# wusize/CLIPSelf

Measured on AMD Instinct MI355X. Metric: images/sec (student+teacher distill step), ViT-B/16 32 crops/img, higher is better.
Workload: dtype bf16; 1 GPU; EVA02-CLIP-B-16 CLIPSelf image-patches step, 64 images x 32 crops per GPU, 224^2 (BASELINE configs[1]); global_batch=64, crops_per_image=32, image_size=224, parallelism=dp1, teacher_chunk=2048, teacher_last_block=cls_query_only, teacher_schedule=one_batch_ahead_on_side_stream

## Files before the change

clipself_amd/csrc/gemm_stream.hip:

```cpp
#include <vector>
#include <cstdio>
#include "gemm_common.h"

namespace {

typedef __attribute__((ext_vector_type(2))) unsigned u32x2;
typedef __attribute__((ext_vector_type(4))) unsigned u32x4;

constexpr unsigned OOB = 0xfffffff0u;

__device__ __forceinline__ float lane_bcast(int src_lane_x4, float v) {
    return __int_as_float(__builtin_amdgcn_ds_bpermute(src_lane_x4, __float_as_int(v)));
}
__device__ __forceinline__ unsigned pack2(float a, float b) {
    union { bf16x2 v; unsigned u; } pk;
    pk.v[0] = f2bf(a);
    pk.v[1] = f2bf(b);
    return pk.u;
}
__device__ __forceinline__ void swap32(unsigned& x, unsigned& y) {
    const u32x2 r = __builtin_amdgcn_permlane32_swap(x, y, false, false);
    x = r[0];
    y = r[1];
}
__device__ __forceinline__ float both_halves(float v) {
    const u32x2 r = __builtin_amdgcn_permlane32_swap(__float_as_uint(v), __float_as_uint(v), false, false);
    return __uint_as_float(r[0]) + __uint_as_float(r[1]);
}
__device__ __forceinline__ __amdgpu_buffer_rsrc_t make_rsrc(const void* base) {
    return __builtin_amdgcn_make_buffer_rsrc(const_cast<void*>(base), 0, 0x7fffffff, 0x00020000);
}
template <int CP>
__device__ __forceinline__ void store16(const u32x4& v, __amdgpu_buffer_rsrc_t rs, unsigned off) {
    __builtin_amdgcn_raw_buffer_store_b128(v, rs, off, 0, CP);
}
template <int CP>
__device__ __forceinline__ void store8(const u32x2& v, __amdgpu_buffer_rsrc_t rs, unsigned off) {
    __builtin_amdgcn_raw_buffer_store_b64(v, rs, off, 0, CP);
}
__device__ __forceinline__ float dot2_bf16(unsigned a, unsigned b, float c) {
    return __builtin_amdgcn_fdot2_f32_bf16(__builtin_bit_cast(bf16x2, a), __builtin_bit_cast(bf16x2, b), c, false);
}
__device__ __forceinline__ float silu_mul(float u, float v) {
    return u * __builtin_amdgcn_rcpf(1.f + __builtin_amdgcn_exp2f(-1.4426950408889634f * u)) * v;
}
template <int ACT>
__device__ __forceinline__ float activate_s(float v) {
    if (ACT == 1) return 0.5f * v * (1.f + erff(v * 0.70710678118654752f));
    if (ACT == 2) return v * __builtin_amdgcn_rcpf(1.f + __builtin_amdgcn_exp2f(-1.702f * 1.4426950408889634f * v));
    return v;
}

struct EpiOps {
    float mean[4], rstd[4];
    float cb, cc;
};

template <bool LN, bool AUX, int CP, int FM = 4>
__device__ __forceinline__ void epi_swiglu(const GemmArgs& p, const f32x16 (&acc)[FM][2], int lane, int row0, int tn, int wn, const EpiOps& eo) {
    const int l31 = lane & 31, hf = lane >> 5;
    const int hbase = tn * 128 + wn * 32;
    const bool colok = hbase < p.group;
    float nm[FM], rs[FM];
#pragma unroll
    for (int i = 0; i < FM; ++i) {
        rs[i] = LN ? eo.rstd[i] : 1.f;
        nm[i] = LN ? -eo.rstd[i] * eo.mean[i] : 0.f;
    }
    unsigned pk[FM][4][2];
    float ssum[4] = {0.f, 0.f, 0.f, 0.f}, ssq[4] = {0.f, 0.f, 0.f, 0.f};
    const int sl0 = hf << 4;
#pragma unroll
    for (int q = 0; q < 4; ++q) {
        float hv[FM][4];
#pragma unroll
        for (int r = 0; r < 4; ++r) {
            const int e = q * 4 + r;
            const int sl = sl0 + ((8 * q + r) << 2);
            const float b1 = lane_bcast(sl, eo.cb), b2 = lane_bcast(sl + 128, eo.cb);
            float c1 = 0.f, c2 = 0.f;
            if (LN) { c1 = lane_bcast(sl, eo.cc); c2 = lane_bcast(sl + 128, eo.cc); }
#pragma unroll
            for (int i = 0; i < FM; ++i) {
                float u = acc[i][0][e], v = acc[i][1][e];
                if (LN) {
                    u = fmaf(rs[i], u, fmaf(nm[i], c1, b1));
                    v = fmaf(rs[i], v, fmaf(nm[i], c2, b2));
                } else {
                    u += b1;
                    v += b2;
                }
                hv[i][r] = silu_mul(u, v);
            }
        }
#pragma unroll
        for (int i = 0; i < FM; ++i) {
            pk[i][q][0] = pack2(hv[i][0], hv[i][1]);
            pk[i][q][1] = pack2(hv[i][2], hv[i][3]);
            if (AUX) {
#pragma unroll
                for (int d = 0; d < 2; ++d) {
                    ssum[i] = dot2_bf16(pk[i][q][d], 0x3f803f80u, ssum[i]);
                    ssq[i] = dot2_bf16(pk[i][q][d], pk[i][q][d], ssq[i]);
                }
            }
        }
    }
    const __amdgpu_buffer_rsrc_t rc = make_rsrc((const __bf16*)p.C + (size_t)row0 * p.ldc + hbase);
#pragma unroll
    for (int i = 0; i < FM; ++i) {
        const bool ok = colok && row0 + i * 32 + l31 < p.M && !CS_ABL(p, 8);
        const unsigned rowoff = (unsigned)((i * 32 + l31) * p.ldc + 8 * hf) * 2u;
#pragma unroll
        for (int pr = 0; pr < 2; ++pr) {
            unsigned x0 = pk[i][2 * pr][0], x1 = pk[i][2 * pr][1], y0 = pk[i][2 * pr + 1][0], y1 = pk[i][2 * pr + 1][1];
            swap32(x0, y0);
            swap32(x1, y1);
            store16<CP>(u32x4{x0, x1, y0, y1}, rc, ok ? rowoff + 32u * pr : OOB);
        }
    }
    if (AUX) {
        const size_t slice = (size_t)tn * 4 + wn;
        const __amdgpu_buffer_rsrc_t rst = make_rsrc(p.stats_part + (slice * p.M + row0) * 2);
#pragma unroll
        for (int i = 0; i < FM; ++i) {
            const float s = both_halves(ssum[i]), q2 = both_halves(ssq[i]);
            const bool ok = colok && hf == 0 && row0 + i * 32 + l31 < p.M;
            store8<CP>(u32x2{__float_as_uint(s), __float_as_uint(q2)}, rst, ok ? (unsigned)(i * 32 + l31) * 8u : OOB);
        }
    }
}

template <int ACT, bool LN, int CP, bool F8 = false, int FM = 4>
__device__ __forceinline__ void epi_bf16(const GemmArgs& p, const f32x16 (&acc)[FM][2], int lane, int row0, int colw, const EpiOps& eo) {
    const int l31 = lane & 31, hf = lane >> 5;
    float nm[FM], rs[FM];
#pragma unroll
    for (int i = 0; i < FM; ++i) {
        rs[i] = (LN || F8) ? eo.rstd[i] : 1.f;
        nm[i] = LN ? -eo.rstd[i] * eo.mean[i] : 0.f;
    }
    const __amdgpu_buffer_rsrc_t rc = make_rsrc((const __bf16*)p.C + (size_t)row0 * p.ldc + colw);
    const int sl0 = hf << 4;
    unsigned pk[2][FM][4][2];
#pragma unroll
    for (int j = 0; j < 2; ++j) {
#pragma unroll
        for (int q = 0; q < 4; ++q) {
            float ov[FM][4];
#pragma unroll
            for (int r = 0; r < 4; ++r) {
                const int sl = sl0 + ((j * 32 + 8 * q + r) << 2);
                const float b = lane_bcast(sl, eo.cb);
                const float c = (LN || F8) ? lane_bcast(sl, eo.cc) : 0.f;
#pragma unroll
                for (int i = 0; i < FM; ++i) {
                    const float a = acc[i][j][q * 4 + r];
                    ov[i][r] = activate_s<ACT>(F8 ? fmaf(rs[i] * c, a, b) : LN ? fmaf(rs[i], a, fmaf(nm[i], c, b)) : a + b);
                }
            }
#pragma unroll
            for (int i = 0; i < FM; ++i) {
                pk[j][i][q][0] = pack2(ov[i][0], ov[i][1]);
                pk[j][i][q][1] = pack2(ov[i][2], ov[i][3]);
            }
        }
    }
#pragma unroll
    for (int i = 0; i < FM; ++i) {
        const bool rowok = row0 + i * 32 + l31 < p.M && !CS_ABL(p, 8);
#pragma unroll
        for (int j = 0; j < 2; ++j) {
            const bool ok = rowok && colw + j * 32 < p.N;
            const unsigned rowoff = (unsigned)((i * 32 + l31) * p.ldc + j * 32 + 8 * hf) * 2u;
#pragma unroll
            for (int pr = 0; pr < 2; ++pr) {
                unsigned x0 = pk[j][i][2 * pr][0], x1 = pk[j][i][2 * pr][1], y0 = pk[j][i][2 * pr + 1][0], y1 = pk[j][i][2 * pr + 1][1];
                swap32(x0, y0);
                swap32(x1, y1);
                store16<CP>(u32x4{x0, x1, y0, y1}, rc, ok ? rowoff + 32u * pr : OOB);
            }
        }
    }
}


template <int ACT, bool LN, int CP>
__device__ __forceinline__ void epi_bf16_slab(const GemmArgs& p, const f32x16 (&acc)[4][2], int lane, int row0, int colw, const EpiOps& eo, char* slab) {
    const int l31 = lane & 31, hf = lane >> 5;
    float nm[4], rs[4];
#pragma unroll
    for (int i = 0; i < 4; ++i) {
        rs[i] = LN ? eo.rstd[i] : 1.f;
        nm[i] = LN ? -eo.rstd[i] * eo.mean[i] : 0.f;
    }
    const __amdgpu_buffer_rsrc_t rc = make_rsrc((const __bf16*)p.C + (size_t)row0 * p.ldc + colw);
    const int sl0 = hf << 4;
    const int piece = lane & 7, col = colw + piece * 8;
#pragma unroll
    for (int half = 0; half < 2; ++half) {
#pragma unroll
        for (int j = 0; j < 2; ++j)
#pragma unroll
            for (int q = 0; q < 4; ++q) {
                float bq[4], cq[4];
#pragma unroll
                for (int r = 0; r < 4; ++r) {
                    const int sl = sl0 + ((j * 32 + 8 * q + r) << 2);
                    bq[r] = lane_bcast(sl, eo.cb);
                    cq[r] = LN ? lane_bcast(sl, eo.cc) : 0.f;
                }
#pragma unroll
                for (int ii = 0; ii < 2; ++ii) {
                    const int i = half * 2 + ii, lrow = ii * 32 + l31;
                    float ov[4];
#pragma unroll
                    for (int r = 0; r < 4; ++r) {
                        const float a = acc[i][j][q * 4 + r];
                        ov[r] = activate_s<ACT>(LN ? fmaf(rs[i], a, fmaf(nm[i], cq[r], bq[r])) : a + bq[r]);
                    }
                    const int s8 = (j * 8 + 2 * q + hf) ^ ((lrow & 7) << 1);
                    *(uint2*)(slab + lrow * 128 + s8 * 8) = make_uint2(pack2(ov[0], ov[1]), pack2(ov[2], ov[3]));
                }
            }
#pragma unroll
        for (int k = 0; k < 8; ++k) {
            const int lrow = (lane >> 3) + 8 * k, rrel = half * 64 + lrow;
            const uint4 w = *(const uint4*)(slab + lrow * 128 + ((piece ^ (lrow & 7)) << 4));
            const bool ok = row0 + rrel < p.M && col < p.N && !CS_ABL(p, 8);
            store16<CP>(u32x4{w.x, w.y, w.z, w.w}, rc, ok ? (unsigned)(rrel * p.ldc + piece * 8) * 2u : OOB);
        }
    }
}

template <bool LN, bool AUX, int CP>
__device__ __forceinline__ void epi_swiglu_slab(const GemmArgs& p, const f32x16 (&acc)[4][2], int lane, int row0, int tn, int wn, const EpiOps& eo,
                                                char* slab) {
    const int l31 = lane & 31, hf = lane >> 5;
    const int hbase = tn * 128 + wn * 32;
    const bool colok = hbase < p.group;
    float nm[4], rs[4];
#pragma unroll
    for (int i = 0; i < 4; ++i) {
        rs[i] = LN ? eo.rstd[i] : 1.f;
        nm[i] = LN ? -eo.rstd[i] * eo.mean[i] : 0.f;
    }
    float ssum[4] = {0.f, 0.f, 0.f, 0.f}, ssq[4] = {0.f, 0.f, 0.f, 0.f};
    const int sl0 = hf << 4;
#pragma unroll
    for (int q = 0; q < 4; ++q) {
        float hv[4][4];
#pragma unroll
        for (int r = 0; r < 4; ++r) {
            const int e = q * 4 + r;
            const int sl = sl0 + ((8 * q + r) << 2);
            const float b1 = lane_bcast(sl, eo.cb), b2 = lane_bcast(sl + 128, eo.cb);
            float c1 = 0.f, c2 = 0.f;
            if (LN) { c1 = lane_bcast(sl, eo.cc); c2 = lane_bcast(sl + 128, eo.cc); }
#pragma unroll
            for (int i = 0; i < 4; ++i) {
                float u = acc[i][0][e], v = acc[i][1][e];
                if (LN) {
                    u = fmaf(rs[i], u, fmaf(nm[i], c1, b1));
                    v = fmaf(rs[i], v, fmaf(nm[i], c2, b2));
// ... 86 lines not shown
                    xin[it][w >> 1][2 * (w & 1)] = __uint_as_float(__builtin_amdgcn_perm(h[w], l[w], 0x05040100u) - 0x8000u);
                    xin[it][w >> 1][2 * (w & 1) + 1] = __uint_as_float(__builtin_amdgcn_perm(h[w], l[w], 0x07060302u) - 0x8000u);
                }
            } else {
                const unsigned off = ok ? (unsigned)(rrel * p.ldc + piece * 8) * 4u : OOB;
                xin[it][0] = __builtin_bit_cast(f32x4, __builtin_amdgcn_raw_buffer_load_b128(rx, off, 0, CP));
                xin[it][1] = __builtin_bit_cast(f32x4, __builtin_amdgcn_raw_buffer_load_b128(rx, ok ? off + 16u : OOB, 0, CP));
            }
        }
        const float rs_row = (LN || F8) ? eo.rstd[i] : 1.f, nm_row = LN ? -eo.rstd[i] * eo.mean[i] : 0.f;
#pragma unroll
        for (int j = 0; j < 2; ++j)
#pragma unroll
            for (int q = 0; q < 4; ++q) {
                f32x4 t;
#pragma unroll
                for (int r = 0; r < 4; ++r) t[r] = acc[i][j][q * 4 + r];
                const int s16 = (j * 8 + 2 * q + hf) ^ (l31 & 15);
                *(f32x4*)(slab + l31 * 256 + s16 * 16) = t;
            }
        EPI_TRACE(1 + 3 * i);
        EPI_TRACE_WAIT();
        EPI_TRACE(2 + 3 * i);
        const int sel = lane & 7;
        float st_s = 0.f, st_q = 0.f;
#pragma unroll
        for (int it = 0; it < 4; ++it) {
            const int lrow = rrow + 8 * it, rrel = i * 32 + lrow;
            const bool ok = colok && row0 + rrel < p.M;
            float rs = 1.f, nm = 0.f;
            if (LN || F8) rs = lane_bcast(lrow << 2, rs_row);
            if (LN) nm = lane_bcast(lrow << 2, nm_row);
            f32x4 o[2];
#pragma unroll
            for (int h = 0; h < 2; ++h) {
                const f32x4 sv = *(const f32x4*)(slab + lrow * 256 + (((2 * piece + h) ^ (lrow & 15)) << 4));
                if (LN) {
#pragma unroll
                    for (int t = 0; t < 4; ++t) o[h][t] = xin[it][h][t] + fmaf(rs, sv[t], fmaf(nm, cc4[h][t], cb4[h][t]));
                } else if (F8) {
#pragma unroll
                    for (int t = 0; t < 4; ++t) o[h][t] = xin[it][h][t] + fmaf(rs * cc4[h][t], sv[t], cb4[h][t]);
                } else {
                    o[h] = xin[it][h] + (sv + cb4[h]);
                }
            }
            if constexpr (SPLIT & 2) {
                const unsigned off = ok ? (unsigned)(rrel * p.ldxb + piece * 8) * 2u : OOB;
                unsigned y[8];
#pragma unroll
                for (int t = 0; t < 8; ++t) y[t] = __float_as_uint(o[t >> 2][t & 3]) + 0x8000u;
                store16<CP>(u32x4{__builtin_amdgcn_perm(y[1], y[0], 0x07060302u), __builtin_amdgcn_perm(y[3], y[2], 0x07060302u),
                                  __builtin_amdgcn_perm(y[5], y[4], 0x07060302u), __builtin_amdgcn_perm(y[7], y[6], 0x07060302u)}, rb, off);
                store16<CP>(u32x4{__builtin_amdgcn_perm(y[1], y[0], 0x05040100u), __builtin_amdgcn_perm(y[3], y[2], 0x05040100u),
                                  __builtin_amdgcn_perm(y[5], y[4], 0x05040100u), __builtin_amdgcn_perm(y[7], y[6], 0x05040100u)}, rl, off);
            } else {
                const unsigned off = ok ? (unsigned)(rrel * p.ldc + piece * 8) * 4u : OOB;
                store16<CP>(__builtin_bit_cast(u32x4, o[0]), rc, off);
                store16<CP>(__builtin_bit_cast(u32x4, o[1]), rc, ok ? off + 16u : OOB);
            }
            if (AUX) {
                if constexpr (!(SPLIT & 2))
                    store16<CP>(u32x4{pack2(o[0][0], o[0][1]), pack2(o[0][2], o[0][3]), pack2(o[1][0], o[1][1]), pack2(o[1][2], o[1][3])}, rb,
                                ok ? (unsigned)(rrel * p.ldxb + piece * 8) * 2u : OOB);
                float ps = 0.f, pq = 0.f;
                if (colok) {
#pragma unroll
                    for (int t = 0; t < 8; ++t) { ps += o[t >> 2][t & 3]; pq = fmaf(o[t >> 2][t & 3], o[t >> 2][t & 3], pq); }
                }
                const float a = sum_lanes8(ps), b = sum_lanes8(pq);
                if (sel == it) { st_s = a; st_q = b; }
            }
        }
        if (AUX) {
            const int rrel = i * 32 + rrow + 8 * sel;
            const bool ok = sel < 4 && row0 + rrel < p.M && colw < p.N;
            store8<CP>(u32x2{__float_as_uint(st_s), __float_as_uint(st_q)}, rst, ok ? (unsigned)rrel * 8u : OOB);
        }
        EPI_TRACE(3 + 3 * i);
        __builtin_amdgcn_sched_barrier(0);
    }
}

template <int EPI, bool AUX, bool SLAB, int SPLIT = 0, int FM = 4>
constexpr int epi_stores() {
    if (EPI == EPI_SWIGLU_BF16) return FM * (2 + (AUX ? 1 : 0));
    if (EPI == EPI_RESID_F32) return FM * (8 + (AUX ? ((SPLIT & 2) ? 0 : 4) + 1 : 0));
    return FM * 4;
}

#ifndef CS_DMA_AUX_A
#define CS_DMA_AUX_A 0
#endif
#ifndef CS_DMA_AUX_B
#define CS_DMA_AUX_B 0
#endif
#define CS_VMCNT(N) asm volatile("s_waitcnt vmcnt(%0)" ::"n"(N) : "memory")

inline bool getenv_flag(const char* name) {
    const char* v = getenv(name);
    return v && v[0] && v[0] != '0';
}

template <int EPI, bool LN, bool AUX, bool SLAB, bool F8 = false, int SPLIT = 0, int BMT = 256>
__global__ __launch_bounds__(512) void gemm_stream_kernel(GemmArgs p) {
    static_assert(BMT == 256 || (BMT == 192 && !F8 && SPLIT == 0 && !LN && !AUX), "192-row tiles: the training schedule's plain epilogues");
    static_assert(SPLIT == 0 || (EPI == EPI_RESID_F32 && LN && !F8), "the split stream belongs to the folded-LayerNorm residual epilogue");
    static_assert(SLAB || EPI != EPI_RESID_F32, "the fp32 residual epilogue exists in the slab form only (whole-line traffic)");
    static_assert(!F8 || (!LN && !AUX && (EPI == EPI_BF16 || EPI == EPI_RESID_F32)), "fp8 operands: bf16 and fp32-residual outputs");
    constexpr int ES = F8 ? 1 : 2;
    constexpr int CP = 0;
    constexpr bool SWI = EPI == EPI_SWIGLU_BF16, RES = EPI == EPI_RESID_F32;
    static_assert(SWI || RES || epi_is_bf16(EPI), "register epilogues");
    constexpr int BM = BMT, BN = 256, WN = 4, TM = BM / 2, TN = 64, FM = TM / 32, FN = 2;
    constexpr int A_BYTES = BM * BK * 2, B_BYTES = BN * BK * 2;
    constexpr int NPA = BM / 32;
    constexpr int NM = FM * FN, NR = FM + FN;
    constexpr int S = epi_stores<EPI, AUX, SLAB, SPLIT, FM>() < 55 ? epi_stores<EPI, AUX, SLAB, SPLIT, FM>() : 55;
    extern __shared__ __attribute__((aligned(16))) char smem[];
    const int tid = threadIdx.x, lane = tid & 63;
    const int wave = __builtin_amdgcn_readfirstlane(tid >> 6);
    const int wm = wave / WN, wn = wave - wm * WN;
    const int hf = lane >> 5, l31 = lane & 31;
    char* const b_ring = smem + 3 * A_BYTES;
    const int ntiles = p.tiles_m * p.tiles_n, ktiles = p.K / (F8 ? 128 : BK);
    const int a_base = ((wm * TM + l31) >> 1) << 8, b_base = ((wn * TN + l31) >> 1) << 8;
    const int par8 = (l31 & 1) << 3, sw = l31 >> 1;
    const int G = gridDim.x;
#ifndef CS_NO_DMA_ROLES
    constexpr bool ROLES = !F8;
#else
    constexpr bool ROLES = false;
#endif
    const bool role_a = ROLES && wave >= 4;
#ifndef CS_NO_MID_BARRIER
    constexpr bool MID = ROLES && !SLAB && !F8;
#else
    constexpr bool MID = false;
#endif

    unsigned avoff[ROLES ? 8 : 4], bvoff[ROLES ? 1 : 4];
    const char *a_src = nullptr, *b_src = nullptr;
    int a_tile = blockIdx.x, a_kt = 0, b_tile = blockIdx.x, b_kt = 0;
    auto set_a = [&](int tile) {
        int tm, tn;
        tile_of_id(p, tile, ntiles, tm, tn);
        a_src = (const char*)p.A + (size_t)tm * BM * p.lda * ES;
#pragma unroll
        for (int i = 0; i < (ROLES ? NPA : 4); ++i) {
            int tr, chk;
            lane_source(ROLES ? (wave & 3) * NPA + i : wave * 4 + i, lane, tr, chk);
            avoff[i] = (unsigned)(min(tr, p.M - 1 - tm * BM) * p.lda * ES + chk * 16);
        }
    };
    auto set_b = [&](int tile) {
        int tm, tn;
        tile_of_id(p, tile, ntiles, tm, tn);
        if (SWI) {
            b_src = (const char*)p.B + (size_t)tn * (BN / 2) * p.ldb * ES;
        } else {
            b_src = (const char*)p.B + (size_t)tn * BN * p.ldb * ES;
        }
#pragma unroll
        for (int i = 0; i < (ROLES ? 8 : 4); ++i) {
            int tr, chk;
            lane_source(ROLES ? (wave & 3) * 8 + i : wave * 4 + i, lane, tr, chk);
            int rel;
            if (SWI) {
                const int hrel = (tr >> 6) * 32 + (tr & 31);
                rel = ((tr >> 5) & 1) * p.group + min(hrel, p.group - 1 - tn * (BN / 2));
            } else {
                rel = min(tr, p.N - 1 - tn * BN);
            }
            (ROLES ? avoff : bvoff)[i] = (unsigned)(rel * p.ldb * ES + chk * 16);
        }
    };
    auto adv_a = [&]() {
        if (++a_kt == ktiles) {
            a_kt = 0;
            if (a_tile + G < ntiles) {
                a_tile += G;
                set_a(a_tile);
            }
        }
    };
    auto adv_b = [&]() {
        if (++b_kt == ktiles) {
            b_kt = 0;
            if (b_tile + G < ntiles) {
                b_tile += G;
                set_b(b_tile);
            }
        }
    };
#define ISSUE_A(X, SLOT)                                                                                                      \
    __builtin_amdgcn_global_load_lds((const __attribute__((address_space(1))) void*)(a_src + (size_t)a_kt * (BK * 2) + avoff[X]), \
                                     (__attribute__((address_space(3))) void*)(smem + (SLOT) * A_BYTES + (wave * 4 + (X)) * 1024), 16, 0, CS_DMA_AUX_A)
#define ISSUE_B(X, SLOT)                                                                                                      \
    __builtin_amdgcn_global_load_lds((const __attribute__((address_space(1))) void*)(b_src + (size_t)b_kt * (BK * 2) + bvoff[X]), \
                                     (__attribute__((address_space(3))) void*)(b_ring + (SLOT) * B_BYTES + (wave * 4 + (X)) * 1024), 16, 0, CS_DMA_AUX_B)

#define ISSUE_RA(X, SLOT)                                                                                                     \
    __builtin_amdgcn_global_load_lds((const __attribute__((address_space(1))) void*)(a_src + (size_t)a_kt * (BK * 2) + avoff[X]), \
                                     (__attribute__((address_space(3))) void*)(smem + (SLOT) * A_BYTES + ((wave & 3) * NPA + (X)) * 1024), 16, 0, CS_DMA_AUX_A)
#define ISSUE_RB(X, SLOT)                                                                                                     \
    __builtin_amdgcn_global_load_lds((const __attribute__((address_space(1))) void*)(b_src + (size_t)b_kt * (BK * 2) + avoff[X]), \
                                     (__attribute__((address_space(3))) void*)(b_ring + (SLOT) * B_BYTES + ((wave & 3) * 8 + (X)) * 1024), 16, 0, CS_DMA_AUX_B)

    if constexpr (ROLES) {
        if (role_a) {
            set_a(a_tile);
#pragma unroll
            for (int x = 0; x < NPA; ++x) ISSUE_RA(x, 0);
            adv_a();
#pragma unroll
            for (int x = 0; x < NPA; ++x) ISSUE_RA(x, 1);
            adv_a();
        } else {
            set_b(b_tile);
#pragma unroll
            for (int x = 0; x < 8; ++x) ISSUE_RB(x, 0);
            adv_b();
            if constexpr (MID) {
#pragma unroll
                for (int x = 0; x < 8; ++x) ISSUE_RB(x, 1);
                adv_b();
            }
        }
        if constexpr (MID) {
            if (role_a) CS_VMCNT(NPA);
            else CS_VMCNT(8);
            __builtin_amdgcn_s_barrier();
        }
    } else {
        set_a(a_tile);
        set_b(b_tile);
#pragma unroll
        for (int x = 0; x < 4; ++x) ISSUE_A(x, 0);
        adv_a();
#pragma unroll
        for (int x = 0; x < 4; ++x) ISSUE_B(x, 0);
        adv_b();
#pragma unroll
        for (int x = 0; x < 4; ++x) ISSUE_A(x, 1);
        adv_a();
    }

    int curA = 0, gpar = 0;
    bool after_epi = false;
    for (int tile = blockIdx.x; tile < ntiles; tile += G) {
        int tm, tn;
        tile_of_id(p, tile, ntiles, tm, tn);
        const int row0 = tm * BM + wm * TM, colw = tn * BN + wn * TN;
        f32x16 acc[FM][FN];
        EpiOps eo;
        auto load_epi_ops = [&](int ln) {
            const int l31 = ln & 31, hf = ln >> 5, lane = ln;
#pragma unroll
            for (int i = 0; i < 4; ++i) eo.mean[i] = eo.rstd[i] = 0.f;
            eo.cb = eo.cc = 0.f;
            if (LN || F8) {
#pragma unroll
                for (int i = 0; i < FM; ++i) {
                    const int r = min(row0 + i * 32 + l31, p.M - 1);
                    if (LN) eo.mean[i] = p.ln_mean[r];
                    eo.rstd[i] = p.ln_rstd[r];
                }
            }
            int co;
            if (SWI) co = hf * p.group + min(tn * 128 + wn * 32 + l31, p.group - 1);
            else co = min(colw + lane, p.N - 1);
            if (!RES) {
                if (p.bias) eo.cb = p.bias[co];
                if (LN || F8) eo.cc = p.ln_colsum[co];
            }
        };

        auto ktile = [&](auto zero_tag, auto role_tag) {
            constexpr bool ZERO = decltype(zero_tag)::value;
            constexpr int ROLE = decltype(role_tag)::value;
            constexpr int KEEP = ROLE == 0 ? 4 : ROLE == 1 ? 0 : NPA;
            constexpr int SS = S + KEEP > 63 ? 63 - KEEP : S;
            if (after_epi) CS_VMCNT(KEEP + SS);
            else CS_VMCNT(KEEP);
            after_epi = false;
            asm volatile("s_waitcnt lgkmcnt(0)" ::: "memory");
            if (!CS_ABL(p, 2))
                __builtin_amdgcn_s_barrier();
            const char* la = smem + curA * A_BYTES + a_base;
            const char* lb = b_ring + gpar * B_BYTES + b_base;
            const int slot_a2 = curA == 0 ? 2 : curA - 1, slot_b1 = gpar ^ 1;
            if constexpr (F8) {
                typedef __attribute__((ext_vector_type(8))) int i32x8;
                typedef __attribute__((ext_vector_type(4))) int i32x4;
#pragma unroll
                for (int s2 = 0; s2 < 2; ++s2) {
                    const int c0 = 4 * s2 + 2 * hf;
                    const int off0 = ((par8 | c0) ^ sw) << 4, off1 = ((par8 | (c0 + 1)) ^ sw) << 4;
                    i32x8 a8[FM], b8[FN];
#pragma unroll
                    for (int i = 0; i < FM; ++i) {
                        const i32x4 lo = *(const i32x4*)(la + i * (16 * 256) + off0), hi = *(const i32x4*)(la + i * (16 * 256) + off1);
                        a8[i] = i32x8{lo[0], lo[1], lo[2], lo[3], hi[0], hi[1], hi[2], hi[3]};
                    }
#pragma unroll
                    for (int j = 0; j < FN; ++j) {
                        const i32x4 lo = *(const i32x4*)(lb + j * (16 * 256) + off0), hi = *(const i32x4*)(lb + j * (16 * 256) + off1);
                        b8[j] = i32x8{lo[0], lo[1], lo[2], lo[3], hi[0], hi[1], hi[2], hi[3]};
                    }
                    if constexpr (ROLE == 1) {
                        if (s2 == 0) {
#pragma unroll
                            for (int x = 0; x < 8; ++x) ISSUE_RB(x, slot_b1);
                        }
                    } else if constexpr (ROLE == 2) {
                        if (s2 == 1) {
#pragma unroll
                            for (int x = 0; x < NPA; ++x) ISSUE_RA(x, slot_a2);
                        }
                    } else if (s2 == 0) {
                        ISSUE_B(0, slot_b1); ISSUE_B(1, slot_b1); ISSUE_B(2, slot_b1); ISSUE_B(3, slot_b1);
                    } else {
                        ISSUE_A(0, slot_a2); ISSUE_A(1, slot_a2); ISSUE_A(2, slot_a2); ISSUE_A(3, slot_a2);
                    }
#pragma unroll
                    for (int i = 0; i < FM; ++i)
#pragma unroll
                        for (int j = 0; j < FN; ++j) {
                            if (ZERO && s2 == 0) {
                                const f32x16 z = {0.f, 0.f, 0.f, 0.f, 0.f, 0.f, 0.f, 0.f, 0.f, 0.f, 0.f, 0.f, 0.f, 0.f, 0.f, 0.f};
                                acc[i][j] = __builtin_amdgcn_mfma_scale_f32_32x32x64_f8f6f4(b8[j], a8[i], z, 0, 0, 0, 0x7f7f7f7f, 0, 0x7f7f7f7f);
                            } else {
                                acc[i][j] = __builtin_amdgcn_mfma_scale_f32_32x32x64_f8f6f4(b8[j], a8[i], acc[i][j], 0, 0, 0, 0x7f7f7f7f, 0, 0x7f7f7f7f);
                            }
                        }
                }
            } else {
                bf16x8 a[2][FM], b[2][FN];
                auto frags = [&](int ks, int buf) {
                    const int off = ((par8 | (ks * 2 + hf)) ^ sw) << 4;
#pragma unroll
                    for (int i = 0; i < FM; ++i) a[buf][i] = *(const bf16x8*)(la + i * (16 * 256) + off);
#pragma unroll
                    for (int j = 0; j < FN; ++j) b[buf][j] = *(const bf16x8*)(lb + j * (16 * 256) + off);
                };
                frags(0, 0);
#ifndef CS_NO_SGB
                __builtin_amdgcn_sched_group_barrier(0x100, 6, 0);
#endif
#pragma unroll
                for (int ks = 0; ks < 4; ++ks) {
                    const int cb = ks & 1;
                    if (ks < 3) frags(ks + 1, cb ^ 1);
// ... 61 lines not shown
            const char* lb = b_ring + gpar * B_BYTES + b_base;
            const char* la_n = smem + nextA * A_BYTES + a_base;
            const char* lb_n = b_ring + (gpar ^ 1) * B_BYTES + b_base;
            const int slot_a2 = curA == 0 ? 2 : curA - 1, slot_b2 = gpar;
            auto frags = [&](const char* pa, const char* pb, int ks, int buf) {
                const int off = ((par8 | (ks * 2 + hf)) ^ sw) << 4;
#pragma unroll
                for (int i = 0; i < FM; ++i) fa[buf][i] = *(const bf16x8*)(pa + i * (16 * 256) + off);
#pragma unroll
                for (int j = 0; j < FN; ++j) fb[buf][j] = *(const bf16x8*)(pb + j * (16 * 256) + off);
            };
            auto mfmas = [&](int cb, bool zero) {
#pragma unroll
                for (int i = 0; i < FM; ++i)
#pragma unroll
                    for (int j = 0; j < FN; ++j) {
                        if (zero) {
                            const f32x16 z = {0.f, 0.f, 0.f, 0.f, 0.f, 0.f, 0.f, 0.f, 0.f, 0.f, 0.f, 0.f, 0.f, 0.f, 0.f, 0.f};
                            acc[i][j] = __builtin_amdgcn_mfma_f32_32x32x16_bf16(fb[cb][j], fa[cb][i], z, 0, 0, 0);
                        } else {
                            acc[i][j] = __builtin_amdgcn_mfma_f32_32x32x16_bf16(fb[cb][j], fa[cb][i], acc[i][j], 0, 0, 0);
                        }
                    }
            };
            if (ZERO) {
                frags(la, lb, 0, 0);
                __builtin_amdgcn_sched_group_barrier(0x100, 6, 0);
            }
#pragma unroll
            for (int ks = 0; ks < 3; ++ks) {
                const int cb = ks & 1;
                frags(la, lb, ks + 1, cb ^ 1);
                constexpr int KA = 1;
                if constexpr (ROLE == 2) {
                    if (ks == KA) {
#pragma unroll
                        for (int x = 0; x < NPA / 2; ++x) ISSUE_RA(x, slot_a2);
                    }
                    if (ks == KA + 1) {
#pragma unroll
                        for (int x = NPA / 2; x < NPA; ++x) ISSUE_RA(x, slot_a2);
                    }
                }
                mfmas(cb, ZERO && ks == 0);
#pragma unroll
                for (int m = 0; m < NM; ++m) {
                    __builtin_amdgcn_sched_group_barrier(0x008, 1, 0);
                    if (m < NR) __builtin_amdgcn_sched_group_barrier(0x100, 1, 0);
                    if (ROLE == 2 && (ks == KA || ks == KA + 1) && m == NM - 2) __builtin_amdgcn_sched_group_barrier(0x010, 2, 0);
                    if (ROLE == 2 && (ks == KA || ks == KA + 1) && m == NM - 1) __builtin_amdgcn_sched_group_barrier(0x010, NPA / 2 - 2, 0);
                }
            }
            {
                constexpr int KEEP = ROLE == 1 ? 0 : NPA;
                constexpr int SS = S + KEEP > 63 ? 63 - KEEP : S;
                if (after_epi) CS_VMCNT(KEEP + SS);
                else CS_VMCNT(KEEP);
                after_epi = false;
                asm volatile("s_waitcnt lgkmcnt(0)" ::: "memory");
                __builtin_amdgcn_s_barrier();
            }
            {
                const int off = ((par8 | hf) ^ sw) << 4;
#pragma unroll
                for (int x = 0; x < 8; ++x) {
                    if (x < FM) fa[0][x] = *(const bf16x8*)(la_n + x * (16 * 256) + off);
                    else if (x < NR) fb[0][x - FM] = *(const bf16x8*)(lb_n + (x - FM) * (16 * 256) + off);
                    if constexpr (ROLE == 1) ISSUE_RB(x, slot_b2);
                }
            }
            mfmas(1, false);
#pragma unroll
            for (int m = 0; m < NM; ++m) {
                __builtin_amdgcn_sched_group_barrier(0x008, 1, 0);
                if (m < NR) __builtin_amdgcn_sched_group_barrier(0x100, 1, 0);
                if (ROLE == 1 && m < NM - 1) __builtin_amdgcn_sched_group_barrier(0x010, 1, 0);
                if (ROLE == 1 && m == NM - 1) __builtin_amdgcn_sched_group_barrier(0x010, 1 + 8 - NM, 0);
            }
            if (ROLE == 1) adv_b();
            else adv_a();
            curA = nextA;
            gpar ^= 1;
        };
        if constexpr (MID) {
            if (role_a) {
                ktile_mid(std::true_type{}, std::integral_constant<int, 2>{});
                for (int kt = 1; kt < ktiles; ++kt) ktile_mid(std::false_type{}, std::integral_constant<int, 2>{});
            } else {
                ktile_mid(std::true_type{}, std::integral_constant<int, 1>{});
                for (int kt = 1; kt < ktiles; ++kt) ktile_mid(std::false_type{}, std::integral_constant<int, 1>{});
            }
        } else if constexpr (ROLES) {
            if (role_a) {
                ktile(std::true_type{}, std::integral_constant<int, 2>{});
                for (int kt = 1; kt < ktiles; ++kt) ktile(std::false_type{}, std::integral_constant<int, 2>{});
            } else {
                ktile(std::true_type{}, std::integral_constant<int, 1>{});
                for (int kt = 1; kt < ktiles; ++kt) ktile(std::false_type{}, std::integral_constant<int, 1>{});
            }
        } else {
            ktile(std::true_type{}, std::integral_constant<int, 0>{});
            for (int kt = 1; kt < ktiles; ++kt) ktile(std::false_type{}, std::integral_constant<int, 0>{});
        }
        if (CS_ABL(p, 4)) continue;
        after_epi = true;
        int lane_e = lane;
        asm volatile("" : "+v"(lane_e));
        if constexpr (SLAB) {
            asm volatile("s_waitcnt lgkmcnt(0)" ::: "memory");
            __builtin_amdgcn_s_barrier();
            char* const slab = wave >= 4 ? b_ring + (gpar ^ 1) * B_BYTES + (wave - 4) * 8192
                               : (BM == 192 && wave == 3) ? b_ring + 2 * B_BYTES
                                                          : smem + (curA == 0 ? 2 : curA - 1) * A_BYTES + wave * 8192;
            load_epi_ops(lane_e);
#ifndef CS_NO_KERNARG_RELOAD
            constexpr bool RELOAD = RES && LN && AUX;
#else
            constexpr bool RELOAD = false;
#endif
            if constexpr (RELOAD) {
                const __attribute__((address_space(4))) GemmArgs* pk = (const __attribute__((address_space(4))) GemmArgs*)__builtin_amdgcn_kernarg_segment_ptr();
                asm volatile("" : "+s"(pk));
                GemmArgs pe;
                pe.A = pk->A; pe.C = pk->C; pe.bias = pk->bias; pe.extra = pk->extra; pe.M = pk->M; pe.N = pk->N; pe.ldc = pk->ldc;
                pe.ln_colsum = pk->ln_colsum; pe.stats_part = pk->stats_part; pe.xb_out = pk->xb_out; pe.ldxb = pk->ldxb; pe.lo = pk->lo;
                pe.dbg = pk->dbg;
                epi_resid_slab<LN, AUX, CP, F8, SPLIT, FM>(pe, acc, lane_e, row0, colw, tn, wn, eo, slab);
            } else if constexpr (RES) {
                epi_resid_slab<LN, AUX, CP, F8, SPLIT, FM>(p, acc, lane_e, row0, colw, tn, wn, eo, slab);
            } else {
                static_assert(FM == 4, "the slab forms of the bf16 / SwiGLU epilogues exist for 256-row tiles");
                if constexpr (SWI) epi_swiglu_slab<LN, AUX, CP>(p, acc, lane_e, row0, tn, wn, eo, slab);
                else epi_bf16_slab<epi_act(EPI), LN, CP>(p, acc, lane_e, row0, colw, eo, slab);
            }
        } else {
            load_epi_ops(lane_e);
            if constexpr (SWI) epi_swiglu<LN, AUX, CP, FM>(p, acc, lane_e, row0, tn, wn, eo);
            else epi_bf16<epi_act(EPI), LN, CP, F8, FM>(p, acc, lane_e, row0, colw, eo);
        }
    }
    CS_VMCNT(0);
#undef ISSUE_A
#undef ISSUE_B
#undef ISSUE_RA
#undef ISSUE_RB
}

template <int EPI, bool LN, bool AUX, bool SLAB, int BMT = 256>
int launch_stream_v(const GemmArgs& a, unsigned grid, hipStream_t stream) {
    constexpr size_t lds = 160 * 1024;
    static bool once = ((void)hipFuncSetAttribute((const void*)gemm_stream_kernel<EPI, LN, AUX, SLAB, false, 0, BMT>, hipFuncAttributeMaxDynamicSharedMemorySize, (int)lds), true);
    (void)once;
    hipLaunchKernelGGL((gemm_stream_kernel<EPI, LN, AUX, SLAB, false, 0, BMT>), dim3(grid), dim3(512), lds, stream, a);
    CS_LAUNCH_CHECK();
    return 0;
}

template <int EPI, bool LN, bool AUX>
int launch_stream_t(const GemmArgs& a, unsigned grid, hipStream_t stream) {
    if constexpr (EPI == EPI_RESID_F32) return launch_stream_v<EPI, LN, AUX, true>(a, grid, stream);
    else return (a.dbg & 1) ? launch_stream_v<EPI, LN, AUX, true>(a, grid, stream) : launch_stream_v<EPI, LN, AUX, false>(a, grid, stream);
}

template <bool AUX, int SPLIT>
int launch_stream_split(const GemmArgs& a, unsigned grid, hipStream_t stream) {
    constexpr size_t lds = 160 * 1024;
    static bool once = ((void)hipFuncSetAttribute((const void*)gemm_stream_kernel<EPI_RESID_F32, true, AUX, true, false, SPLIT>,
                                                  hipFuncAttributeMaxDynamicSharedMemorySize, (int)lds), true);
    (void)once;
    hipLaunchKernelGGL((gemm_stream_kernel<EPI_RESID_F32, true, AUX, true, false, SPLIT>), dim3(grid), dim3(512), lds, stream, a);
    CS_LAUNCH_CHECK();
    return 0;
}

template <int EPI>
int launch_stream_bf16(const GemmArgs& a, unsigned grid, hipStream_t stream) {
    return a.ln_mean ? launch_stream_t<EPI, true, false>(a, grid, stream) : launch_stream_t<EPI, false, false>(a, grid, stream);
}

template <int EPI, bool SLAB>
int launch_stream_f8(const GemmArgs& a, unsigned grid, hipStream_t stream) {
    constexpr size_t lds = 160 * 1024;
    static bool once = ((void)hipFuncSetAttribute((const void*)gemm_stream_kernel<EPI, false, false, SLAB, true>, hipFuncAttributeMaxDynamicSharedMemorySize, (int)lds), true);
    (void)once;
    hipLaunchKernelGGL((gemm_stream_kernel<EPI, false, false, SLAB, true>), dim3(grid), dim3(512), lds, stream, a);
    CS_LAUNCH_CHECK();
    return 0;
}

}

int cs_gemm_stream_launch_f8(GemmArgs a, int epi, int reserve, hipStream_t stream) {
    a.tiles_m = (a.M + 255) / 256;
    a.tiles_n = (a.N + 255) / 256;
    const long ntiles = (long)a.tiles_m * a.tiles_n;
    const long cap = cs_persistent_cap(reserve);
    const unsigned grid = (unsigned)(ntiles < cap ? ntiles : cap);
    if (epi == EPI_BF16) return launch_stream_f8<EPI_BF16, false>(a, grid, stream);
    return launch_stream_f8<EPI_RESID_F32, true>(a, grid, stream);
}

#ifdef CS_ABLATION_SWITCHES
static int stream_launch_impl(GemmArgs a, int epi, int reserve, hipStream_t stream);
int cs_gemm_stream_launch(GemmArgs a, int epi, int reserve, hipStream_t stream) {
    static const char* path = getenv("CS_GEMM_TRACE");
    static unsigned long long* buf = nullptr;
    constexpr size_t WORDS = 256 * 8 * 16;
    if (path && !buf && hipMalloc((void**)&buf, WORDS * 8) == hipSuccess) {
        (void)hipMemset(buf, 0, WORDS * 8);
        (void)hipMemcpyToSymbol(HIP_SYMBOL(g_epi_trace), &buf, sizeof(buf));
    }
    const int rc = stream_launch_impl(a, epi, reserve, stream);
    if (path && buf && rc == 0 && (epi == EPI_RESID_F32 || epi == EPI_RESID_LN_F32)) {
        (void)hipStreamSynchronize(stream);
        std::vector<unsigned long long> host(WORDS);
        (void)hipMemcpy(host.data(), buf, WORDS * 8, hipMemcpyDeviceToHost);
        if (FILE* f = fopen(path, "wb")) { fwrite(host.data(), 8, WORDS, f); fclose(f); }
    }
    return rc;
}
static int stream_launch_impl(GemmArgs a, int epi, int reserve, hipStream_t stream) {
#else
int cs_gemm_stream_launch(GemmArgs a, int epi, int reserve, hipStream_t stream) {
#endif
    const bool swi = epi == EPI_SWIGLU_BF16, res = epi == EPI_RESID_F32 || epi == EPI_RESID_LN_F32;
    if (!(swi || res || epi == EPI_BF16 || epi == EPI_QGELU_BF16)) return 1;
    if (a.M < 1 || a.K % BK != 0) return 1;
    if (swi ? (a.group % 32 != 0) : (a.N % 32 != 0)) return 1;
    if ((long)a.ldc * 128 * 4 >= 0x70000000L || (long)a.ldxb * 128 * 2 >= 0x70000000L) return 1;
    const bool ln = a.ln_mean != nullptr;
    if ((epi == EPI_RESID_LN_F32) != (res && ln)) return 1;
    bool aux = false;
    if (swi) aux = a.stats_part != nullptr;
    else if (res) {
        if ((a.stats_part != nullptr) != (a.xb_out != nullptr)) return 1;
        aux = a.stats_part != nullptr;
        if (aux && (a.ldxb % 8 != 0 || ((uintptr_t)a.xb_out % 16) != 0)) return 1;
    } else if (a.stats_part || a.xb_out) return 1;
    a.tiles_m = (a.M + 255) / 256;
    a.tiles_n = swi ? (a.group + 127) / 128 : (a.N + 255) / 256;
    long ntiles = (long)a.tiles_m * a.tiles_n;
    const long cap = cs_persistent_cap(reserve);
    unsigned grid = (unsigned)(ntiles < cap ? ntiles : cap);
    if (!ln && !aux && !(a.dbg & 1) && a.M >= 192 && (swi || res || epi == EPI_BF16) && !getenv_flag("CS_NO_BM192")) {
// ... 78 lines not shown
```

Baseline: 743.6 images/sec.

## Use 16x16x32 MFMA main loop for folded-LN bf16 and SwiGLU GEMMs

Adds a variant of the streaming GEMM kernel whose inner loop uses 16x16x32 bf16 MFMA instructions instead of the 32x32 form. It comes with new register epilogues for the folded-LayerNorm bf16 and SwiGLU outputs that work on the 16-row fragment layout, using permlane16 swaps. This variant becomes the default for those epilogues, and an environment flag restores the old path. The aim is better MFMA throughput and scheduling on MI355X for these GEMMs. The cost is more fragment loads from LDS and more registers spent on accumulators.

```diff
diff --git a/clipself_amd/csrc/gemm_stream.hip b/clipself_amd/csrc/gemm_stream.hip
--- a/clipself_amd/csrc/gemm_stream.hip
+++ b/clipself_amd/csrc/gemm_stream.hip
@@ -23,6 +23,11 @@
     x = r[0];
     y = r[1];
 }
+__device__ __forceinline__ void swap16(unsigned& x, unsigned& y) {
+    const u32x2 r = __builtin_amdgcn_permlane16_swap(x, y, false, false);
+    x = r[0];
+    y = r[1];
+}
 __device__ __forceinline__ float both_halves(float v) {
     const u32x2 r = __builtin_amdgcn_permlane32_swap(__float_as_uint(v), __float_as_uint(v), false, false);
     return __uint_as_float(r[0]) + __uint_as_float(r[1]);
@@ -51,10 +56,12 @@
     return v;
 }
 
-struct EpiOps {
-    float mean[4], rstd[4];
+template <int NB>
+struct EpiOpsT {
+    float mean[NB], rstd[NB];
     float cb, cc;
 };
+typedef EpiOpsT<4> EpiOps;
 
 template <bool LN, bool AUX, int CP, int FM = 4>
 __device__ __forceinline__ void epi_swiglu(const GemmArgs& p, const f32x16 (&acc)[FM][2], int lane, int row0, int tn, int wn, const EpiOps& eo) {
@@ -180,6 +187,146 @@
                 swap32(x1, y1);
                 store16<CP>(u32x4{x0, x1, y0, y1}, rc, ok ? rowoff + 32u * pr : OOB);
             }
+        }
+    }
+}
+
+template <int ACT, bool LN, int CP>
+__device__ __forceinline__ void epi_bf16_m16(const GemmArgs& p, const f32x4 (&acc)[8][4], int lane, int row0, int colw, const EpiOpsT<8>& eo) {
+    const int l15 = lane & 15, g = lane >> 4;
+    float nm[8], rs[8];
+#pragma unroll
+    for (int i = 0; i < 8; ++i) {
+        rs[i] = LN ? eo.rstd[i] : 1.f;
+        nm[i] = LN ? -eo.rstd[i] * eo.mean[i] : 0.f;
+    }
+    const __amdgpu_buffer_rsrc_t rc = make_rsrc((const __bf16*)p.C + (size_t)row0 * p.ldc + colw);
+    const int sl0 = g << 4;
+    unsigned pk[4][8][2];
+#pragma unroll
+    for (int j = 0; j < 4; ++j) {
+        float b[4], c[4];
+#pragma unroll
+        for (int r = 0; r < 4; ++r) {
+            const int sl = sl0 + ((j * 16 + r) << 2);
+            b[r] = lane_bcast(sl, eo.cb);
+            c[r] = LN ? lane_bcast(sl, eo.cc) : 0.f;
+        }
+#pragma unroll
+        for (int i = 0; i < 8; ++i) {
+            float ov[4];
+#pragma unroll
+            for (int r = 0; r < 4; ++r) ov[r] = activate_s<ACT>(LN ? fmaf(rs[i], acc[i][j][r], fmaf(nm[i], c[r], b[r])) : acc[i][j][r] + b[r]);
+            pk[j][i][0] = pack2(ov[0], ov[1]);
+            pk[j][i][1] = pack2(ov[2], ov[3]);
+        }
+        __builtin_amdgcn_sched_barrier(0);
+    }
+#pragma unroll
+    for (int t = 0; t < 4; ++t) {
+        const int rrel = (2 * t + (g & 1)) * 16 + l15;
+        const bool rowok = row0 + rrel < p.M && !CS_ABL(p, 8);
+#pragma unroll
+        for (int j = 0; j < 4; ++j) {
+            const bool ok = rowok && colw + j * 16 < p.N;
+            unsigned x0 = pk[j][2 * t][0], x1 = pk[j][2 * t][1], y0 = pk[j][2 * t + 1][0], y1 = pk[j][2 * t + 1][1];
+            swap16(x0, y0);
+            swap16(x1, y1);
+            store16<CP>(u32x4{x0, x1, y0, y1}, rc, ok ? (unsigned)(rrel * p.ldc + j * 16 + 8 * (g >> 1)) * 2u : OOB);
+        }
+    }
+}
+
+template <bool LN, bool AUX, int CP>
+__device__ __forceinline__ void epi_swiglu_m16(const GemmArgs& p, const f32x4 (&acc)[8][4], int lane, int row0, int tn, int wn, const EpiOpsT<8>& eo) {
+    const int l15 = lane & 15, g = lane >> 4;
+    const int hbase = tn * 128 + wn * 32;
+    const bool colok = hbase < p.group;
+    float nm[8], rs[8];
+#pragma unroll
+    for (int i = 0; i < 8; ++i) {
+        rs[i] = LN ? eo.rstd[i] : 1.f;
+        nm[i] = LN ? -eo.rstd[i] * eo.mean[i] : 0.f;
+    }
+    unsigned pk[2][8][2];
+    float ssum[8] = {0.f, 0.f, 0.f, 0.f, 0.f, 0.f, 0.f, 0.f}, ssq[8] = {0.f, 0.f, 0.f, 0.f, 0.f, 0.f, 0.f, 0.f};
+    const int sl0 = g << 4;
+#pragma unroll
+    for (int j = 0; j < 2; ++j) {
+        float b1[4], b2[4], c1[4], c2[4];
+#pragma unroll
+        for (int r = 0; r < 4; ++r) {
+            const int sl = sl0 + ((j * 16 + r) << 2);
+            b1[r] = lane_bcast(sl, eo.cb);
+            b2[r] = lane_bcast(sl + 128, eo.cb);
+            c1[r] = LN ? lane_bcast(sl, eo.cc) : 0.f;
+            c2[r] = LN ? lane_bcast(sl + 128, eo.cc) : 0.f;
+        }
+#pragma unroll
+        for (int i = 0; i < 8; ++i) {
+            float hv[4];
+#pragma unroll
+            for (int r = 0; r < 4; ++r) {
+                float u = acc[i][j][r], v = acc[i][j + 2][r];
+                if (LN) {
+                    u = fmaf(rs[i], u, fmaf(nm[i], c1[r], b1[r]));
+                    v = fmaf(rs[i], v, fmaf(nm[i], c2[r], b2[r]));
+                } else {
+                    u += b1[r];
+                    v += b2[r];
+                }
+                hv[r] = silu_mul(u, v);
+            }
+            pk[j][i][0] = pack2(hv[0], hv[1]);
+            pk[j][i][1] = pack2(hv[2], hv[3]);
+            if (AUX) {
+#pragma unroll
+                for (int d = 0; d < 2; ++d) {
+                    ssum[i] = dot2_bf16(pk[j][i][d], 0x3f803f80u, ssum[i]);
+                    ssq[i] = dot2_bf16(pk[j][i][d], pk[j][i][d], ssq[i]);
+                }
+            }
+        }
+    }
+    const __amdgpu_buffer_rsrc_t rc = make_rsrc((const __bf16*)p.C + (size_t)row0 * p.ldc + hbase);
+#pragma unroll
+    for (int t = 0; t < 4; ++t) {
+        const int rrel = (2 * t + (g & 1)) * 16 + l15;
+        const bool ok = colok && row0 + rrel < p.M && !CS_ABL(p, 8);
+#pragma unroll
+        for (int j = 0; j < 2; ++j) {
+            unsigned x0 = pk[j][2 * t][0], x1 = pk[j][2 * t][1], y0 = pk[j][2 * t + 1][0], y1 = pk[j][2 * t + 1][1];
+            swap16(x0, y0);
+            swap16(x1, y1);
+            store16<CP>(u32x4{x0, x1, y0, y1}, rc, ok ? (unsigned)(rrel * p.ldc + j * 16 + 8 * (g >> 1)) * 2u : OOB);
+        }
+    }
+    if (AUX) {
+        const size_t slice = (size_t)tn * 4 + wn;
+        const __amdgpu_buffer_rsrc_t rst = make_rsrc(p.stats_part + (slice * p.M + row0) * 2);
+        auto reduce = [&](const float (&v)[8], float (&out)[2]) {
+            unsigned h[4];
+#pragma unroll
+            for (int b = 0; b < 4; ++b) {
+                unsigned x = __float_as_uint(v[b]), y = __float_as_uint(v[b + 4]);
+                swap32(x, y);
+                h[b] = __float_as_uint(__uint_as_float(x) + __uint_as_float(y));
+            }
+#pragma unroll
+            for (int k = 0; k < 2; ++k) {
+                unsigned x = h[k], y = h[k + 2];
+                swap16(x, y);
+                out[k] = __uint_as_float(x) + __uint_as_float(y);
+            }
+        };
+        float s[2], q2[2];
+        reduce(ssum, s);
+        reduce(ssq, q2);
+#pragma unroll
+        for (int k = 0; k < 2; ++k) {
+            const int rrel = (2 * g + k) * 16 + l15;
+            const bool ok = colok && row0 + rrel < p.M;
+            store8<CP>(u32x2{__float_as_uint(s[k]), __float_as_uint(q2[k])}, rst, ok ? (unsigned)rrel * 8u : OOB);
         }
     }
 }
@@ -432,8 +579,9 @@
     }
 }
 
-template <int EPI, bool AUX, bool SLAB, int SPLIT = 0, int FM = 4>
+template <int EPI, bool AUX, bool SLAB, int SPLIT = 0, int FM = 4, int MF = 32>
 constexpr int epi_stores() {
+    if (EPI == EPI_SWIGLU_BF16 && MF == 16) return 8 + (AUX ? 2 : 0);
     if (EPI == EPI_SWIGLU_BF16) return FM * (2 + (AUX ? 1 : 0));
     if (EPI == EPI_RESID_F32) return FM * (8 + (AUX ? ((SPLIT & 2) ? 0 : 4) + 1 : 0));
     return FM * 4;
@@ -452,8 +600,11 @@
     return v && v[0] && v[0] != '0';
 }
 
-template <int EPI, bool LN, bool AUX, bool SLAB, bool F8 = false, int SPLIT = 0, int BMT = 256>
+template <int EPI, bool LN, bool AUX, bool SLAB, bool F8 = false, int SPLIT = 0, int BMT = 256, int MF = 32>
 __global__ __launch_bounds__(512) void gemm_stream_kernel(GemmArgs p) {
+    static_assert(MF == 32 || (MF == 16 && LN && !SLAB && !F8 && SPLIT == 0 && BMT == 256 && (epi_is_bf16(EPI) ? !AUX : EPI == EPI_SWIGLU_BF16)),
+                  "16x16x32 loop: the folded-LN bf16 and SwiGLU register epilogues");
+    constexpr bool M16 = MF == 16;
     static_assert(BMT == 256 || (BMT == 192 && !F8 && SPLIT == 0 && !LN && !AUX), "192-row tiles: the training schedule's plain epilogues");
     static_assert(SPLIT == 0 || (EPI == EPI_RESID_F32 && LN && !F8), "the split stream belongs to the folded-LayerNorm residual epilogue");
     static_assert(SLAB || EPI != EPI_RESID_F32, "the fp32 residual epilogue exists in the slab form only (whole-line traffic)");
@@ -466,12 +617,12 @@
     constexpr int A_BYTES = BM * BK * 2, B_BYTES = BN * BK * 2;
     constexpr int NPA = BM / 32;
     constexpr int NM = FM * FN, NR = FM + FN;
-    constexpr int S = epi_stores<EPI, AUX, SLAB, SPLIT, FM>() < 55 ? epi_stores<EPI, AUX, SLAB, SPLIT, FM>() : 55;
+    constexpr int S = epi_stores<EPI, AUX, SLAB, SPLIT, FM, MF>() < 55 ? epi_stores<EPI, AUX, SLAB, SPLIT, FM, MF>() : 55;
     extern __shared__ __attribute__((aligned(16))) char smem[];
     const int tid = threadIdx.x, lane = tid & 63;
     const int wave = __builtin_amdgcn_readfirstlane(tid >> 6);
     const int wm = wave / WN, wn = wave - wm * WN;
-    const int hf = lane >> 5, l31 = lane & 31;
+    const int hf = M16 ? lane >> 4 : lane >> 5, l31 = M16 ? lane & 15 : lane & 31;
     char* const b_ring = smem + 3 * A_BYTES;
     const int ntiles = p.tiles_m * p.tiles_n, ktiles = p.K / (F8 ? 128 : BK);
     const int a_base = ((wm * TM + l31) >> 1) << 8, b_base = ((wn * TN + l31) >> 1) << 8;
@@ -602,23 +753,25 @@
         int tm, tn;
         tile_of_id(p, tile, ntiles, tm, tn);
         const int row0 = tm * BM + wm * TM, colw = tn * BN + wn * TN;
-        f32x16 acc[FM][FN];
-        EpiOps eo;
+        f32x16 acc[M16 ? 1 : FM][M16 ? 1 : FN];
+        f32x4 acc16[M16 ? 8 : 1][M16 ? 4 : 1];
+        constexpr int RB = M16 ? 16 : 32, NRB = TM / RB;
+        EpiOpsT<M16 ? 8 : 4> eo;
         auto load_epi_ops = [&](int ln) {
-            const int l31 = ln & 31, hf = ln >> 5, lane = ln;
-#pragma unroll
-            for (int i = 0; i < 4; ++i) eo.mean[i] = eo.rstd[i] = 0.f;
+            const int l31 = ln & (RB - 1), hf = ln >> 5, lane = ln;
+#pragma unroll
+            for (int i = 0; i < (M16 ? 8 : 4); ++i) eo.mean[i] = eo.rstd[i] = 0.f;
             eo.cb = eo.cc = 0.f;
             if (LN || F8) {
 #pragma unroll
-                for (int i = 0; i < FM; ++i) {
-                    const int r = min(row0 + i * 32 + l31, p.M - 1);
+                for (int i = 0; i < NRB; ++i) {
+                    const int r = min(row0 + i * RB + l31, p.M - 1);
                     if (LN) eo.mean[i] = p.ln_mean[r];
                     eo.rstd[i] = p.ln_rstd[r];
                 }
             }
             int co;
-            if (SWI) co = hf * p.group + min(tn * 128 + wn * 32 + l31, p.group - 1);
+            if (SWI) co = hf * p.group + min(tn * 128 + wn * 32 + (lane & 31), p.group - 1);
             else co = min(colw + lane, p.N - 1);
             if (!RES) {
                 if (p.bias) eo.cb = p.bias[co];
@@ -846,7 +999,111 @@
             curA = nextA;
             gpar ^= 1;
         };
-        if constexpr (MID) {
+        bf16x8 ga[2][M16 ? 4 : 1], gb[M16 ? 4 : 1];
+        auto ktile_m16 = [&](auto zero_tag, auto role_tag) {
+            constexpr bool ZERO = decltype(zero_tag)::value;
+            constexpr int ROLE = decltype(role_tag)::value;
+            const int nextA = curA == 2 ? 0 : curA + 1;
+            const char* la = smem + curA * A_BYTES + a_base;
+            const char* lb = b_ring + gpar * B_BYTES + b_base;
+            const char* la_n = smem + nextA * A_BYTES + a_base;
+            const char* lb_n = b_ring + (gpar ^ 1) * B_BYTES + b_base;
+            const int slot_a2 = curA == 0 ? 2 : curA - 1, slot_b2 = gpar;
+            auto frag = [&](const char* base, int ks, int blk) {
+                const int off = (((par8 | (ks * 4 + hf)) ^ sw) << 4) ^ ((blk & 1) << 7);
+                return *(const bf16x8*)(base + blk * (8 * 256) + off);
+            };
+            auto read_a = [&](const char* pa, int ks, int c) {
+#pragma unroll
+                for (int x = 0; x < 4; ++x) ga[c][x] = frag(pa, ks, c * 4 + x);
+            };
+            auto read_b = [&](const char* pb, int ks, int jj) {
+                gb[2 * jj] = frag(pb, ks, 2 * jj);
+                gb[2 * jj + 1] = frag(pb, ks, 2 * jj + 1);
+            };
+            auto mfmas = [&](int c, int jj, bool zero) {
+#pragma unroll
+                for (int x = 0; x < 4; ++x)
+#pragma unroll
+                    for (int j = 2 * jj; j < 2 * jj + 2; ++j) {
+                        if (zero) {
+                            const f32x4 z = {0.f, 0.f, 0.f, 0.f};
+                            acc16[c * 4 + x][j] = __builtin_amdgcn_mfma_f32_16x16x32_bf16(gb[j], ga[c][x], z, 0, 0, 0);
+                        } else {
+                            acc16[c * 4 + x][j] = __builtin_amdgcn_mfma_f32_16x16x32_bf16(gb[j], ga[c][x], acc16[c * 4 + x][j], 0, 0, 0);
+                        }
+                    }
+            };
+            auto order = [&](auto r0a, auto nra, auto r0b, auto nrb, auto d0a, auto nda, auto d0b, auto ndb) {
+#pragma unroll
+                for (int m = 0; m < 16; ++m) {
+                    __builtin_amdgcn_sched_group_barrier(0x008, 1, 0);
+                    if ((m >= r0a.value && m < r0a.value + nra.value) || (m >= r0b.value && m < r0b.value + nrb.value))
+                        __builtin_amdgcn_sched_group_barrier(0x100, 1, 0);
+                    if ((m >= d0a.value && m < d0a.value + nda.value) || (m >= d0b.value && m < d0b.value + ndb.value))
+                        __builtin_amdgcn_sched_group_barrier(0x010, 1, 0);
+                }
+            };
+#define CI(N) std::integral_constant<int, (N)>{}
+            if (ZERO) {
+                read_a(la, 0, 0);
+                read_b(lb, 0, 0);
+                __builtin_amdgcn_sched_group_barrier(0x100, 6, 0);
+            }
+            read_b(lb, 0, 1);
+            mfmas(0, 0, ZERO);
+            read_a(la, 0, 1);
+            mfmas(0, 1, ZERO);
+            order(CI(0), CI(2), CI(8), CI(4), CI(0), CI(0), CI(0), CI(0));
+            read_a(la, 1, 0);
+            mfmas(1, 0, ZERO);
+            read_b(lb, 1, 0);
+            if constexpr (ROLE == 2) {
+#pragma unroll
+                for (int x = 0; x < NPA / 2; ++x) ISSUE_RA(x, slot_a2);
+            }
+            mfmas(1, 1, ZERO);
+            order(CI(0), CI(4), CI(8), CI(2), CI(10), CI(ROLE == 2 ? NPA / 2 : 0), CI(0), CI(0));
+            read_b(lb, 1, 1);
+            if constexpr (ROLE == 2) {
+#pragma unroll
+                for (int x = NPA / 2; x < NPA; ++x) ISSUE_RA(x, slot_a2);
+            }
+            mfmas(0, 0, false);
+            read_a(la, 1, 1);
+            mfmas(0, 1, false);
+            order(CI(0), CI(2), CI(8), CI(4), CI(2), CI(ROLE == 2 ? NPA / 2 : 0), CI(0), CI(0));
+            {
+                constexpr int KEEP = ROLE == 1 ? 0 : NPA;
+                constexpr int SS = S + KEEP > 63 ? 63 - KEEP : S;
+                if (after_epi) CS_VMCNT(KEEP + SS);
+                else CS_VMCNT(KEEP);
+                after_epi = false;
+                asm volatile("s_waitcnt lgkmcnt(0)" ::: "memory");
+                __builtin_amdgcn_s_barrier();
+            }
+            read_a(la_n, 0, 0);
+            if constexpr (ROLE == 1) { ISSUE_RB(0, slot_b2); ISSUE_RB(1, slot_b2); ISSUE_RB(2, slot_b2); ISSUE_RB(3, slot_b2); }
+            mfmas(1, 0, false);
+            read_b(lb_n, 0, 0);
+            if constexpr (ROLE == 1) { ISSUE_RB(4, slot_b2); ISSUE_RB(5, slot_b2); ISSUE_RB(6, slot_b2); ISSUE_RB(7, slot_b2); }
+            mfmas(1, 1, false);
+            order(CI(0), CI(4), CI(8), CI(2), CI(4), CI(ROLE == 1 ? 4 : 0), CI(10), CI(ROLE == 1 ? 4 : 0));
+#undef CI
+            if (ROLE == 1) adv_b();
+            else adv_a();
+            curA = nextA;
+            gpar ^= 1;
+        };
+        if constexpr (M16) {
+            if (role_a) {
+                ktile_m16(std::true_type{}, std::integral_constant<int, 2>{});
+                for (int kt = 1; kt < ktiles; ++kt) ktile_m16(std::false_type{}, std::integral_constant<int, 2>{});
+            } else {
+                ktile_m16(std::true_type{}, std::integral_constant<int, 1>{});
+                for (int kt = 1; kt < ktiles; ++kt) ktile_m16(std::false_type{}, std::integral_constant<int, 1>{});
+            }
+        } else if constexpr (MID) {
             if (role_a) {
                 ktile_mid(std::true_type{}, std::integral_constant<int, 2>{});
                 for (int kt = 1; kt < ktiles; ++kt) ktile_mid(std::false_type{}, std::integral_constant<int, 2>{});
@@ -899,7 +1156,9 @@
             }
         } else {
             load_epi_ops(lane_e);
-            if constexpr (SWI) epi_swiglu<LN, AUX, CP, FM>(p, acc, lane_e, row0, tn, wn, eo);
+            if constexpr (M16 && SWI) epi_swiglu_m16<LN, AUX, CP>(p, acc16, lane_e, row0, tn, wn, eo);
+            else if constexpr (M16) epi_bf16_m16<epi_act(EPI), LN, CP>(p, acc16, lane_e, row0, colw, eo);
+            else if constexpr (SWI) epi_swiglu<LN, AUX, CP, FM>(p, acc, lane_e, row0, tn, wn, eo);
             else epi_bf16<epi_act(EPI), LN, CP, F8, FM>(p, acc, lane_e, row0, colw, eo);
         }
     }
@@ -910,12 +1169,12 @@
 #undef ISSUE_RB
 }
 
-template <int EPI, bool LN, bool AUX, bool SLAB, int BMT = 256>
+template <int EPI, bool LN, bool AUX, bool SLAB, int BMT = 256, int MF = 32>
 int launch_stream_v(const GemmArgs& a, unsigned grid, hipStream_t stream) {
     constexpr size_t lds = 160 * 1024;
-    static bool once = ((void)hipFuncSetAttribute((const void*)gemm_stream_kernel<EPI, LN, AUX, SLAB, false, 0, BMT>, hipFuncAttributeMaxDynamicSharedMemorySize, (int)lds), true);
+    static bool once = ((void)hipFuncSetAttribute((const void*)gemm_stream_kernel<EPI, LN, AUX, SLAB, false, 0, BMT, MF>, hipFuncAttributeMaxDynamicSharedMemorySize, (int)lds), true);
     (void)once;
-    hipLaunchKernelGGL((gemm_stream_kernel<EPI, LN, AUX, SLAB, false, 0, BMT>), dim3(grid), dim3(512), lds, stream, a);
+    hipLaunchKernelGGL((gemm_stream_kernel<EPI, LN, AUX, SLAB, false, 0, BMT, MF>), dim3(grid), dim3(512), lds, stream, a);
     CS_LAUNCH_CHECK();
     return 0;
 }
@@ -923,7 +1182,11 @@
 template <int EPI, bool LN, bool AUX>
 int launch_stream_t(const GemmArgs& a, unsigned grid, hipStream_t stream) {
     if constexpr (EPI == EPI_RESID_F32) return launch_stream_v<EPI, LN, AUX, true>(a, grid, stream);
-    else return (a.dbg & 1) ? launch_stream_v<EPI, LN, AUX, true>(a, grid, stream) : launch_stream_v<EPI, LN, AUX, false>(a, grid, stream);
+    else if (a.dbg & 1) return launch_stream_v<EPI, LN, AUX, true>(a, grid, stream);
+    else if constexpr (LN && (epi_is_bf16(EPI) ? !AUX : EPI == EPI_SWIGLU_BF16)) {
+        if (!getenv_flag("CS_GEMM_MFMA32")) return launch_stream_v<EPI, LN, AUX, false, 256, 16>(a, grid, stream);
+        return launch_stream_v<EPI, LN, AUX, false>(a, grid, stream);
+    } else return launch_stream_v<EPI, LN, AUX, false>(a, grid, stream);
 }
 
 template <bool AUX, int SPLIT>
```

Result: faster. 759.9 images/sec, median of 6 (+2.2%).
